# Koukyosyumei/MyZKP

Hardware: AMD Instinct MI355X
Metric: G1 MSM pairs/sec + NTT elems/sec at 2^20 and 2^24; bit-exact vs CPU (higher is better)
Workload: dtype u32x9 (29-bit limbs, 254-bit Montgomery); 1 GPU; KZG commit = BN254 G1 Pippenger MSM of 2^20 (scalar, point) pairs per GPU against a device-resident SRS (commit_kzg, kzg.rs:57-59); 17-bit signed windows (library default at this size), 15 window tables built once at upload; N GPUs = one MSM of N*2^20 pairs (BASELINE configs[2]/[3]); pairs_per_gpu=1048576, seed=332211571536, window_bits=17

## Files before the change

myzkp_amd/csrc/mzk_api.hip:

```cpp
#include <stdarg.h>
#include <stdlib.h>
#include <atomic>
#include "mzk_common.h"
#include "mzk_gl.h"

namespace mzk {

static thread_local char g_err[512] = "";
void set_error(const char* fmt, ...) {
  va_list ap;
  va_start(ap, fmt);
  vsnprintf(g_err, sizeof g_err, fmt, ap);
  va_end(ap);
}
void clear_error() { g_err[0] = 0; }
int hip_fail(hipError_t e, const char* what, const char* file, int line) {
  set_error("HIP error %d (%s) in %s at %s:%d", (int)e, hipGetErrorString(e), what, file, line);
  return MZK_E_HIP;
}

static std::atomic<uint64_t> g_owner{0};
static thread_local int t_depth = 0;
static thread_local char t_marker;
EntryGuard::EntryGuard() : ok(true), nested(false) {
// ... 1028 lines not shown
    const bool last = k == nc - 1;
    if (!last && g_table_budget && bytes > g_table_budget) continue;
    void* p = nullptr;
    if (n == 0 || dev_alloc(&p, bytes, "SRS handle") == MZK_OK) {
      h->d_points_mont = p; h->has_tables = cand[k].tables; h->window_bits = cand[k].bits; h->sets = cand[k].sets;
      return MZK_OK;
    }
  }
  set_error("SRS handle: the device has no %zu bytes left for the prepared points alone (idle workspace already released)", n * 128);
  return MZK_E_NOMEM;
}
int srs_fill(mzk_srs* h, const void* d_plain, hipStream_t s) {
  WsFrame ws("srs_fill");
  const size_t n = h->n;
  if (n == 0) return MZK_OK;
  if (!h->has_tables) return msm_prepare_points(d_plain, n, h->d_points_mont, (uint8_t*)h->d_points_mont + n * 64, s);
  void* d_mont;
  MZK_TRY(ws.get(WS_MSM_POINTS, n * 64, &d_mont));
  MZK_TRY(msm_prepare_points(d_plain, n, d_mont, nullptr, s));
  return msm_build_tables(d_mont, n, h->d_points_mont, h->window_bits * h->sets, s);
}
}

extern "C" {

int mzk_set_table_budget(size_t bytes) { g_table_budget = bytes; return MZK_OK; }
int mzk_set_workspace_budget(size_t bytes) {
  MZK_ENTER();
  g_ws_budget = bytes;
  if (bytes) {
// ... 486 lines not shown
```

myzkp_amd/csrc/mzk_common.h:

```cpp
#pragma once
#include <hip/hip_runtime.h>
#include <stdint.h>
#include <stddef.h>
#include <stdio.h>
#include <string.h>
#include <functional>
#include <string>
#include <vector>
#include "../../include/mzk.h"
#include "mzk_field.h"
#include "mzk_msm_plan.h"
#include "mzk_ws.h"

namespace mzk {

#ifdef MZK_TUNING
#include <stdlib.h>
static inline int tune_int(const char* name, int dflt) { const char* v = getenv(name); return v ? atoi(v) : dflt; } static inline const char* tune_str(const char* name) { return getenv(name); }
#else
static inline constexpr int tune_int(const char*, int dflt) { return dflt; }
static inline constexpr const char* tune_str(const char*) { return nullptr; }
#endif

void set_error(const char* fmt, ...);
// ... 167 lines not shown
  int k, K;
  size_t i0;
  size_t n_total;
  size_t n_alloc;
};
struct MsmChunk { const void* d_scalars; size_t i0, n; hipEvent_t ready; };
int msm_chunked_impl(const MsmChunk* chunks, int K, const void* d_points, size_t n_total, int point_kind, size_t table_stride, void* d_out,
                     bool out_partial_xyzz, hipStream_t s, const std::function<int(int)>* before_chunk = nullptr);
bool msm_chunkable(size_t n_total, int point_kind, size_t table_stride);
int msm_dev_impl(const void* d_scalars, const void* d_points, size_t n, int point_kind, size_t table_stride, void* d_out,
                 bool out_partial_xyzz, hipStream_t s, const std::function<int()>* points_ready = nullptr, const MsmChunkCtx* cc = nullptr);

bool msm_many_supported(int window_bits);
int msm_generic_window_bits(size_t n);
int msm_many_dev_impl(const void* d_scalars, size_t n, size_t stride_elems, size_t count, const void* d_tables, int c, size_t table_stride, void* d_out,
                      hipStream_t s);
constexpr size_t MSM_DIRECT_MAX_N = (size_t)1 << 14;
size_t msm_direct_bytes(size_t n, int c);
int msm_build_direct(const void* d_points_mont, size_t n, int c, void* d_direct, hipStream_t s);
int msm_direct_many_dev_impl(const void* d_scalars, size_t n, size_t stride_elems, size_t count, const void* d_direct, int c, size_t table_stride, void* d_out,
                             hipStream_t s);

int xyzz_batch_to_affine(const void* d_xyzz, size_t count, void* d_out, bool out_mont, hipStream_t s);
int msm_build_tables(const void* d_points_mont, size_t n, void* d_tables, int window_bits, hipStream_t s);
int msm_fold_partials_impl(const void* d_partials, int count, void* d_out_xy, hipStream_t s);
int msm_prepare_points(const void* d_points_plain, size_t n, void* d_points_mont, void* d_phi, hipStream_t s);
int msm_phi_points(const void* d_points_mont, size_t n, void* d_phi, hipStream_t s);
int synth_field_impl(int fid, uint64_t seed, size_t n, void* d_out, hipStream_t s);
int synth_g1_impl(uint64_t seed, size_t n, void* d_out, hipStream_t s);
int selftest_inv_wave_impl(uint64_t seed, size_t n, uint64_t* mismatches_host, hipStream_t s);
int selftest_row_ec_impl(uint64_t seed, size_t n, int dbl_reps, uint64_t* mismatches_host, hipStream_t s);
// ... 18 lines not shown
}

struct mzk_srs {
  void* d_points_mont;
  size_t n;
  bool has_tables;
  int window_bits;
  int ctx_index;
  int sets = 1;
  void* d_direct = nullptr;
  int direct_bits = 0;
  size_t direct_bytes = 0;
  mutable void* d_tables_wide = nullptr;
  mutable int wide_bits = 0;
  mutable size_t wide_bytes = 0;
  int kind() const { return has_tables ? (mzk::MSM_PTS_TABLES | (window_bits << 8) | (sets << 16)) : (int)mzk::MSM_PTS_MONT; }
  size_t table_rows() const { return has_tables ? (size_t)mzk::msm_table_rows(window_bits, sets) : 2; }
};

namespace mzk {
bool srs_many_capable(const mzk_srs* srs);
int msm_many_srs(const mzk_srs* srs, const void* d_scalars, size_t n, size_t stride_elems, size_t count, void* d_out, hipStream_t s,
                 size_t shift = 0);
bool kzg_open_many_supported(const mzk_srs* srs, size_t n);
int kzg_open_many_dev(const mzk_srs* srs, const void* d_coefs, size_t n, size_t count, const uint64_t* us_host, void* d_ys, void* d_ws_xy, hipStream_t s);
}
```

myzkp_amd/csrc/mzk_io.hip:

```cpp
#include <stdio.h>
#include <vector>
#include "mzk_common.h"

using namespace mzk;

namespace mzk {
int srs_alloc_layout(mzk_srs* h, int with_tables);
struct SrsFileHeader {
  char magic[8];
  uint32_t format;
  uint32_t flags;
  uint64_t n;
  uint32_t window_bits;
  uint32_t table_rows;
  uint64_t points_fnv1a;
  uint64_t tables_fnv1a;
  uint64_t reserved[2];
};
static_assert(sizeof(SrsFileHeader) == 64, "header layout");
static const char SRS_MAGIC[8] = {'M', 'Z', 'K', 'S', 'R', 'S', 0, 0};
static const size_t IO_CHUNK_POINTS = (size_t)1 << 19;

static uint64_t fnv1a(uint64_t h, const void* data, size_t len) {
  const uint8_t* p = (const uint8_t*)data;
// ... 83 lines not shown
  if (hash != h.points_fnv1a) { set_error("srs_load: checksum mismatch in %s (corrupted or truncated)", path); return MZK_E_IO; }
  const int want_bits = with_tables > 1 ? with_tables : msm_srs_window_bits(n);
  const bool use_stored = with_tables && h.format >= 2 && (h.flags & 1u) && (int)h.window_bits == want_bits &&
                          h.table_rows == (uint32_t)(msm_table_windows(want_bits) - 1) && n > 0;
  if (!use_stored) return mzk_srs_from_device_ex(d_plain, n, with_tables, out, s);
  WsGuard wsg(s);
  mzk_srs* hd = new mzk_srs{nullptr, n, false, 0, ctx().index};
  const size_t rows = (size_t)h.table_rows + 1;
  int rc = srs_alloc_layout(hd, with_tables);
  if (rc == MZK_OK && !(hd->has_tables && hd->sets == 1 && hd->window_bits == want_bits)) {
    mzk_srs_free(hd);
    return mzk_srs_from_device_ex(d_plain, n, with_tables, out, s);
  }
  if (rc != MZK_OK) { delete hd; return rc; }
  uint64_t thash = hash;
  if (rc == MZK_OK) rc = msm_prepare_points(d_plain, n, hd->d_points_mont, nullptr, s);
  for (size_t row = 1; rc == MZK_OK && row < rows; row++) {
    for (size_t at = 0; rc == MZK_OK && at < n; at += IO_CHUNK_POINTS) {
      const size_t m = n - at < IO_CHUNK_POINTS ? n - at : IO_CHUNK_POINTS;
      if (fread(host.data(), 64, m, fc.f) != m) { set_error("srs_load: %s is truncated (tables)", path); rc = MZK_E_IO; break; }
      thash = fnv1a_words(thash, host.data(), m * 64);
      if (hipMemcpyAsync((uint8_t*)hd->d_points_mont + (row * n + at) * 64, host.data(), m * 64, hipMemcpyHostToDevice, s) != hipSuccess ||
          hipStreamSynchronize(s) != hipSuccess) { set_error("srs_load: copy failed"); rc = MZK_E_HIP; }
    }
  }
  if (rc == MZK_OK && hipStreamSynchronize(s) != hipSuccess) rc = MZK_E_HIP;
  if (rc == MZK_OK && thash != h.tables_fnv1a) { set_error("srs_load: checksum mismatch in the window tables of %s (corrupted or stale)", path); rc = MZK_E_IO; }
  if (rc != MZK_OK) { mzk_srs_free(hd); return rc; }
  *out = hd;
  return MZK_OK;
// ... 24 lines not shown
```

myzkp_amd/csrc/mzk_msm.hip:

```cpp
#include <stdlib.h>
#include <type_traits>
#include "mzk_common.h"
#include "mzk_elem.h"
#include "mzk_ec.h"
#include "mzk_coop.h"
#include "mzk_row.h"
#include "mzk_glv.h"
#include "mzk_affine_wave.h"

namespace mzk {

static const MsmKnobs& msm_knobs() {
  static const MsmKnobs k = [] {
    const MsmKnobs d;
    return MsmKnobs{tune_int("MZK_GLV_C", d.glv_c), tune_int("MZK_SMALL_SCAN", d.small_scan), tune_int("MZK_SCAN_MAX_LOG", d.scan_max_log),
                    tune_int("MZK_ACC_SEG", d.acc_seg), tune_int("MZK_COARSE_LOG_20", d.coarse_log_20),
                    tune_int("MZK_COARSE_LOG_17", d.coarse_log_17), tune_int("MZK_PER_FINE", d.per_fine), tune_int("MZK_SORT_SCAN_FREE", d.sort_scan_free),
                    tune_int("MZK_COMBINE_WIDE_MIN_LOG", d.combine_wide_min_log)};
  }();
  return k;
}

int msm_generic_window_bits(size_t n) { return choose_shape_glv(n ? n : 1, msm_knobs().glv_c).c; }

// ... 704 lines not shown
    hipLaunchKernelGGL(k_scan_finish, dim3((unsigned)((n + 255) / 256 + 1)), dim3(256), 0, s, out, (const u32*)scratch, sb, n);
  } else {
    MZK_TRY(launch_exclusive_scan((const u32*)scratch, scratch, sb, scratch + sb + 2, s));
    hipLaunchKernelGGL(k_scan_add, dim3((unsigned)(n / 256 + 1)), dim3(256), 0, s, out, (const u32*)scratch, sb, n);
  }
  MZK_HIP(hipGetLastError());
  return MZK_OK;
}

constexpr u32 SEG_MIN = 8;
__device__ __forceinline__ u32 segment_length(u32 seg_host, u32 t_max, u32 total_entries) {
  if (t_max == 0) return seg_host;
  const u32 v = (total_entries + t_max - 1) / t_max;
  return v < SEG_MIN ? SEG_MIN : v;
}
template <bool SENT = false>
__global__ __launch_bounds__(256, 3) void k_seg_accumulate(const u32* __restrict__ points_mont, const u32* __restrict__ offsets,
                                                         const u32* __restrict__ entries, u32* __restrict__ slots, size_t nbuckets,
                                                         u32 seg_host, u32 t_max) {
  const size_t t = (size_t)blockIdx.x * blockDim.x + threadIdx.x;
  const u32 total_entries = offsets[nbuckets];
  u32 e0, e1;
  if (!seg_span(t, segment_length(seg_host, t_max, total_entries), total_entries, &e0, &e1)) return;
  const auto offset_at = [&](size_t b) __attribute__((always_inline)) { return offsets[b]; };
  Xyzz acc = xyzz_inf();
  u32 w[16];
  Affine pt;
  bool skip = false;
  seg_walk<SENT>(
      e0, e1, seg_first_bucket(offset_at, nbuckets, e0), nbuckets, [&](u32 e) __attribute__((always_inline)) { return entries[e]; }, offset_at,
      [&](u32 ref) __attribute__((always_inline)) {
        const size_t idx = ref & 0x7fffffffu;
        load_words8(points_mont + idx * 16, w);
        load_words8(points_mont + idx * 16 + 8, w + 8);
      },
      [&](u32 ent) __attribute__((always_inline)) {
#pragma unroll
        for (int k = 0; k < 16; k++) asm volatile("" : "+v"(w[k]));
        skip = affine_words_is_inf(w) || (SENT && ent == MANY_SENTINEL);
        pt = affine_load_mont(w);
      },
      [&](size_t b) __attribute__((always_inline)) {
        xyzz_gstore_raw(slots, t + b, acc);
        acc = xyzz_inf();
      },
      [&](u32, u32 ent, size_t) __attribute__((always_inline)) {
        if (!skip) acc = xyzz_madd_signed_with<FeAsm>(acc, pt, (ent >> 31) != 0);
      });
}
constexpr u32 HEAVY_SLOTS_SORT1 = 16;
__device__ __forceinline__ u32 bucket_end(const u32* __restrict__ offsets, const u32* __restrict__ tails, int lg_nb, size_t b) {
  if (tails && (b & (((size_t)1 << lg_nb) - 1)) == (((size_t)1 << lg_nb) - 1)) return tails[b >> lg_nb];
  return offsets[b + 1];
}
__device__ __forceinline__ bool defer_heavy(size_t b, size_t s0, size_t s1, u32 o1, u32* __restrict__ heavy, bool leader, u32 threshold = HEAVY_SLOTS) {
  if (s1 - s0 + 1 <= threshold) return false;
  if (leader) { const u32 i = atomicAdd(&heavy[0], 1u); heavy[HEAVY_HDR + 2 * i] = (u32)b; heavy[HEAVY_HDR + 2 * i + 1] = o1; }
  return true;
}
__global__ __launch_bounds__(128) void k_seg_combine_wide(const u32* __restrict__ slots, const u32* __restrict__ offsets,
                                                           u32* __restrict__ buckets, size_t nbuckets, u32 seg_host, u32* __restrict__ heavy, u32 t_max) {
  const size_t b = (size_t)blockIdx.x * blockDim.x + threadIdx.x;
  if (b >= nbuckets) return;
// ... 337 lines not shown
  }
  MZK_TRY(launch_reduce_tail_row(buckets, lgB, t_start, sets, wsum, 0, s));
  MZK_HIP(hipGetLastError());
  prof_end(s, MZK_PH_MSM_REDUCE);
  prof_begin(s, MZK_PH_MSM_COMBINE);
  MZK_TRY(launch_window_combine_row((const u32*)wsum, sets, horner_c, out_partial_xyzz ? 1 : 0, d_out, s));
  prof_end(s, MZK_PH_MSM_COMBINE);
  return MZK_OK;
}

int msm_prepare_points(const void* d_points_plain, size_t n, void* d_points_mont, void* d_phi, hipStream_t s) {
  if (n == 0) return MZK_OK;
  hipLaunchKernelGGL(k_prepare_points, dim3((unsigned)((n + 255) / 256)), dim3(256), 0, s, (const u32*)d_points_plain,
                     (u32*)d_points_mont, n, (u32*)d_phi);
  MZK_HIP(hipGetLastError());
  return MZK_OK;
}
int msm_points_to_plain(const void* d_points_mont, size_t n, void* d_points_plain, hipStream_t s) {
  if (n == 0) return MZK_OK;
  hipLaunchKernelGGL(k_points_to_plain, dim3((unsigned)((n + 255) / 256)), dim3(256), 0, s, (const u32*)d_points_mont, n, (u32*)d_points_plain);
  MZK_HIP(hipGetLastError());
  return MZK_OK;
}
int msm_phi_points(const void* d_points_mont, size_t n, void* d_phi, hipStream_t s) {
  if (n == 0) return MZK_OK;
  hipLaunchKernelGGL(k_phi_points, dim3((unsigned)((n + 255) / 256)), dim3(256), 0, s, (const u32*)d_points_mont, n, (u32*)d_phi);
  MZK_HIP(hipGetLastError());
  return MZK_OK;
}

// ... 175 lines not shown
      hipLaunchKernelGGL(k_wg_hist_prefix, dim3((unsigned)((P.NB + 255) / 256)), dim3(256), 0, s, wghist, P.nwg, (int)P.NB, counts);
      MZK_TRY(launch_exclusive_scan((const u32*)counts, offsets, P.NB, scan, s));
      hipLaunchKernelGGL(k_digits_scatter_lds, dim3(P.nwg), dim3(LDS_SORT_THREADS), lds, s, (const u32*)d_scalars, n, P.per_wg, P.L, (const u32*)offsets,
                         (const u32*)wghist, (const u32*)ranks, entries);
    } else {
      const unsigned nblk = (unsigned)((n + 255) / 256);
      MZK_HIP(hipMemsetAsync(counts, 0, P.NB * 4, s));
      hipLaunchKernelGGL(k_digits_count, dim3(nblk), dim3(256), 0, s, (const u32*)d_scalars, n, P.L, counts, ranks);
      MZK_TRY(launch_exclusive_scan((const u32*)counts, offsets, P.NB, scan, s));
      hipLaunchKernelGGL(k_digits_scatter, dim3(nblk), dim3(256), 0, s, (const u32*)d_scalars, n, P.L, offsets, ranks, entries);
    }
    MZK_HIP(hipGetLastError());
    prof_end(s, MZK_PH_MSM_SORT);
    MZK_TRY(prepare());
    prof_begin(s, MZK_PH_MSM_ACCUMULATE);
    hipLaunchKernelGGL(k_seg_accumulate<false>, dim3((unsigned)((P.T + 255) / 256)), dim3(256), 0, s, pts, offsets, entries, slots, P.NB, P.seg, P.t_max);
    prof_end(s, MZK_PH_MSM_ACCUMULATE);
    prof_begin(s, MZK_PH_MSM_SEG_COMBINE);
    if (P.combine_wide)
      hipLaunchKernelGGL(k_seg_combine_wide, dim3((unsigned)((P.NB + 127) / 128)), dim3(128), 0, s, slots, offsets, buckets, P.NB, P.seg, heavy, P.t_max);
    else
      hipLaunchKernelGGL(k_seg_combine, dim3((unsigned)((4 * P.NB + 127) / 128)), dim3(128), 0, s, slots, offsets, buckets, P.NB, P.seg, heavy, (const u32*)nullptr, 0, P.t_max);
    hipLaunchKernelGGL(k_seg_combine_heavy, dim3(HEAVY_GRID), dim3(HEAVY_THREADS), 0, s, (const u32*)slots, (const u32*)offsets, buckets, heavy, P.max_heavy);
    MZK_HIP(hipGetLastError());
    prof_end(s, MZK_PH_MSM_SEG_COMBINE);
    if (cc) return MZK_OK;
  }
  MZK_TRY(reduce_bucket_sets(buckets, P.lgB, P.red_windows, P.one_set, P.horner_c, wsum, (u32*)d_out, out_partial_xyzz, s));
  MZK_HIP(hipGetLastError());
  return MZK_OK;
}
// ... 140 lines not shown
  if (j + 1 == npoly && tid == 0) offsets[npoly * NB] = (u32)(npoly * cap);
  if (tid == 0) tails[j] = base + total;
  __syncthreads();
#pragma unroll
  for (int k = 0; k < SORT1_PER_LANE; k++) {
    const size_t i = tid + (size_t)k * SORT1_THREADS;
    if (i < n) walk_digits_merged<C>(w[k], table_stride, i, [&](int, u32 key, u32 payload) { stage[counter_inc_agg(hist, key)] = payload; });
  }
  __syncthreads();
  for (u32 e = tid; e < cap; e += SORT1_THREADS) entries[base + e] = (e < total) ? stage[e] : MANY_SENTINEL;
}

bool msm_many_supported(int window_bits) { return window_bits == 8 || (window_bits >= 10 && window_bits <= 13); }

int msm_many_dev_impl(const void* d_scalars, size_t n, size_t stride_elems, size_t count, const void* d_tables, int c, size_t table_stride, void* d_out,
                      hipStream_t s) {
  if (count == 0) return MZK_OK;
  if (!d_out || ((!d_scalars || !d_tables) && n)) { set_error("msm_many: null pointer"); return MZK_E_ARG; }
  if (!msm_many_supported(c)) { set_error("msm_many: window width %d has no grid-batched path", c); return MZK_E_ARG; }
  if (n == 0) {
    MZK_HIP(hipMemsetAsync(d_out, 0, count * 64, s));
    return MZK_OK;
  }
  const int nwin = msm_table_windows(c), lgB = c - 1;
  const size_t NB = (size_t)1 << lgB;
  if ((size_t)nwin * table_stride > ((size_t)1 << 31)) { set_error("msm_many: table rows exceed the 31-bit point references"); return MZK_E_ARG; }
  const int nch = (int)((n + MANY_CHUNK - 1) / MANY_CHUNK);
  size_t per_pass = ((size_t)1 << 21) / NB;
  const size_t by_coefs = (((size_t)1 << 22) + n - 1) / n;
  if (by_coefs < per_pass) per_pass = by_coefs;
  if (per_pass < 1) per_pass = 1;
// ... 43 lines not shown
        hipLaunchKernelGGL((k_many_sort1<C>), dim3(nwg), dim3(SORT1_THREADS), n * (size_t)nwin * 4, s, sc, n, stride_elems * 8, table_stride,       \
                           (u32)(n * (size_t)nwin), offs, cnt, entries, tails);                                                                           \
        break;                                                                                                                                       \
      }                                                                                                                                              \
      hipLaunchKernelGGL((k_many_count<C>), dim3(nwg), dim3(MANY_THREADS), 0, s, sc, n, stride_elems * 8, nch, offs);                                \
      MZK_TRY(launch_exclusive_scan((const u32*)offs, offs, ncnt, scan_tmp, s));                                                                     \
      hipLaunchKernelGGL((k_many_scatter<C>), dim3(nwg), dim3(MANY_THREADS), 0, s, sc, n, stride_elems * 8, nch, table_stride, (const u32*)offs,     \
                         nch > 1 ? compact : (u32*)nullptr, NBtot, entries);                                                                         \
      break;
    switch (c) { MZK_MANY_CASE(8) MZK_MANY_CASE(10) MZK_MANY_CASE(11) MZK_MANY_CASE(12) MZK_MANY_CASE(13) }
#undef MZK_MANY_CASE
    MZK_HIP(hipGetLastError());
    prof_end(s, MZK_PH_MSM_SORT);
    prof_begin(s, MZK_PH_MSM_ACCUMULATE);
    const u32 t_max = one_kernel_sort ? 0u : (u32)T;
    if (one_kernel_sort)
      hipLaunchKernelGGL(k_seg_accumulate<true>, dim3((unsigned)((T + 255) / 256)), dim3(256), 0, s, (const u32*)d_tables, (const u32*)compact, (const u32*)entries,
                         slots, NBtot, seg, t_max);
    else
      hipLaunchKernelGGL(k_seg_accumulate<false>, dim3((unsigned)((T + 255) / 256)), dim3(256), 0, s, (const u32*)d_tables, (const u32*)compact, (const u32*)entries,
                         slots, NBtot, seg, t_max);
    prof_end(s, MZK_PH_MSM_ACCUMULATE);
    prof_begin(s, MZK_PH_MSM_SEG_COMBINE);
    const unsigned cgrid = (unsigned)((4 * NBtot + 127) / 128);
    hipLaunchKernelGGL(k_seg_combine, dim3(cgrid), dim3(128), 0, s, slots, (const u32*)compact, buckets, NBtot, seg, heavy, (const u32*)tails, lgB, t_max);
    hipLaunchKernelGGL(k_seg_combine_heavy, dim3(HEAVY_GRID), dim3(HEAVY_THREADS), 0, s, (const u32*)slots, (const u32*)compact, buckets, heavy, max_heavy);
    MZK_HIP(hipGetLastError());
    prof_end(s, MZK_PH_MSM_SEG_COMBINE);
    prof_begin(s, MZK_PH_MSM_REDUCE);
    int t_start = 0;
    MZK_TRY(launch_halving_steps(buckets, lgB, (int)cnt, row_tail_max_ops(), &t_start, s));
    MZK_TRY(launch_reduce_tail_row(buckets, lgB, t_start, (int)cnt, out, 1, s));
    MZK_HIP(hipGetLastError());
    prof_end(s, MZK_PH_MSM_REDUCE);
  }
  return MZK_OK;
// ... 166 lines not shown
    if (!srs->d_tables_wide && srs->wide_bits == 0) {
      const size_t bytes = (size_t)msm_table_windows(MANY_WIDE_BITS) * srs->n * 64;
      const size_t own = (size_t)srs->n * 64 * srs->table_rows() + srs->direct_bytes;
      void* t = nullptr;
      const bool within_budget = table_budget_bytes() == 0 || own + bytes <= table_budget_bytes();
      if (within_budget && dev_alloc(&t, bytes, "wide window tables of the grid-batched pass") == MZK_OK) {
        const int rc = msm_build_tables(srs->d_points_mont, srs->n, t, MANY_WIDE_BITS, s);
        if (rc != MZK_OK) { (void)ws_hook_free(t); return rc; }
        srs->d_tables_wide = t; srs->wide_bits = MANY_WIDE_BITS; srs->wide_bytes = bytes;
      } else {
        srs->wide_bits = -1;
        if (within_budget) clear_error();
      }
    }
    if (srs->d_tables_wide)
      return msm_many_dev_impl(d_scalars, n, stride_elems, count, (const char*)srs->d_tables_wide + shift * 64, srs->wide_bits, srs->n, d_out, s);
  }
  return msm_many_dev_impl(d_scalars, n, stride_elems, count, (const char*)srs->d_points_mont + shift * 64, srs->window_bits, srs->n, d_out, s);
}

int msm_fold_partials_impl(const void* d_partials, int count, void* d_out_xy, hipStream_t s) {
  if (!d_partials || !d_out_xy || count < 0) { set_error("fold_partials: bad argument"); return MZK_E_ARG; }
  MZK_TRY(launch_fold_partials_row((const u32*)d_partials, count, (u32*)d_out_xy, s));
  return MZK_OK;
}

}

namespace mzk {
__device__ __forceinline__ u64 splitmix64(u64& s) {
  u64 z = (s += 0x9e3779b97f4a7c15ULL);
  z = (z ^ (z >> 30)) * 0xbf58476d1ce4e5b9ULL;
  z = (z ^ (z >> 27)) * 0x94d049bb133111ebULL;
// ... 91 lines not shown
```

myzkp_amd/csrc/mzk_msm_plan.h:

```cpp
#pragma once
#include <stddef.h>
#include <stdint.h>
#include <stdio.h>
#include "../../include/mzk.h"

namespace mzk {

enum { MSM_PTS_PLAIN = 0, MSM_PTS_MONT = 1, MSM_PTS_TABLES = 2 };
static inline int msm_table_windows(int c) { return 254 / c + 1; }
static inline int msm_table_rows(int c, int sets) { return 254 / (c * sets) + 1; }

constexpr int SCALAR_BITS = 254;
constexpr int MAX_WINDOWS = 32;
constexpr int GLV_MAG_BITS = 126;
constexpr int SLOT_WORDS = 36;
constexpr int ACC_RESIDENT_WAVES = 3;

struct DigitLayout {
  int c, nwin, merged;
  int sets;
  size_t table_stride;
  int glv;
  size_t phi_offset;
};
// ... 64 lines not shown
  int err = MZK_OK;
  char msg[192] = {};
  size_t n = 0;
  DigitLayout L{};
  int lgB = 0, red_windows = 0, horner_c = 0;
  size_t NB = 0, NBtot = 0;
  bool one_set = false, small_wide = false;
  MsmPath path = MsmPath::SmallSort;
  int cl = 0, F = 0, fb = 0, key_shift = 0, S = 0, nwg = 0;
  uint32_t fine_mask = 0, slice_cap = 0;
  unsigned fine_wgs = 0;
  size_t per_wg = 0;
  bool compact = false, coarse_free = false, fine_free = false, scatter_staged = false;
  int coarse_c = 0;
  uint32_t seg = 0, t_max = 0;
  size_t T = 0, nslots = 0, max_heavy = 0, slot_region_words = 0;
  bool combine_wide = false;
  MsmSizing own{}, alloc{};
  MsmWsBytes ws{}, ws_used{};
  MsmPlan& fail(const char* fmt, size_t a = 0, size_t b = 0, size_t c = 0) { err = MZK_E_ARG; snprintf(msg, sizeof msg, fmt, a, b, c); return *this; }
};

static inline size_t msm_slot_region_words(size_t T, size_t NB) {
  return ((T + NB + 1) * SLOT_WORDS + heavy_total_words((T + NB) / HEAVY_SLOTS + 1) + 3) & ~(size_t)3;
}
static inline MsmPlan& msm_sized(MsmPlan& P, size_t regions) {
  for (int u = 0; u < 2; u++) {
    const MsmSizing& z = u ? P.own : P.alloc;
    MsmWsBytes& w = u ? P.ws_used : P.ws;
    w.points = P.ws.points, w.out = P.ws.out;
    w.offsets = regions * (P.NBtot + 1) * 4;
    w.entries = regions * z.E * 4;
    w.buckets = regions * P.NB * 128;
    if (P.path == MsmPath::SmallScan || P.path == MsmPath::SmallSort) continue;
    const bool two = P.path == MsmPath::TwoLevel;
    w.counts = 2 * P.NBtot * 4;
    w.cursor = z.E * (two ? 8 : 4);
// ... 33 lines not shown
  if (!chunks && (scan_ok || n < (L.merged ? SMALL_MAX_N : SMALL_MAX_N - 1)) && P.NB <= SMALL_MAX_BUCKETS) {
    P.path = scan_ok ? MsmPath::SmallScan : MsmPath::SmallSort;
    P.small_wide = E_max / P.NB > 64;
    return msm_sized(P, 1);
  }
  const size_t ref_max = L.merged ? (size_t)msm_table_rows(L.c, L.sets) * table_stride : L.phi_offset + n;
  if (ref_max > ((size_t)1 << 31) || E_max >= ((size_t)1 << 32))
    return P.fail("msm: %zu pairs x %zu windows (table stride %zu) exceed the 31-bit point references / 32-bit entry offsets", n, (size_t)L.nwin, table_stride);

  const size_t resident_lanes = (size_t)num_cu * 4 * ACC_RESIDENT_WAVES * 64;
  size_t seg = (E_max + resident_lanes - 1) / resident_lanes;
  seg = kn.acc_seg > 0 ? (size_t)kn.acc_seg : seg < 16 ? 16 : seg;
  P.seg = (uint32_t)seg;
  P.T = P.own.T = (E_max + seg - 1) / seg;
  P.t_max = kn.acc_seg > 0 ? 0u : (uint32_t)P.T;
  P.nslots = P.T + P.NB + 1;
  P.max_heavy = (P.T + P.NB) / HEAVY_SLOTS + 1;
  P.combine_wide = P.NB >= ((size_t)1 << kn.combine_wide_min_log);
  const size_t T_seg = E_alloc / (kn.acc_seg > 0 ? (size_t)kn.acc_seg : 16) + 1;
  P.alloc.T = !chunks ? P.T : kn.acc_seg > 0 ? T_seg : (resident_lanes + 1 < T_seg ? resident_lanes + 1 : T_seg);
  P.slot_region_words = msm_slot_region_words(P.alloc.T, P.NB);

  const bool plain_merged = L.merged && L.sets == 1;
  P.cl = (plain_merged && L.c == 20 && kn.coarse_log_20 == 10) ? 10 : COARSE_LOG;
  if (plain_merged && L.c == 17 && kn.coarse_log_17 == 9 && COARSE_LOG == 8 && ref_max > ((size_t)1 << (31 - 8)) && ref_max <= ((size_t)1 << (31 - 7)))
    P.cl = 9;
  if (L.glv && P.NBtot > ((size_t)STAGE_F_MAX << COARSE_LOG)) P.cl = 10;
  const size_t cbins = (size_t)1 << P.cl;
  const bool two_level = (P.NBtot & (P.NBtot - 1)) == 0 && P.NBtot >= 4096 && (P.NBtot / cbins) <= (size_t)FINE_MAX &&
                         (n >= 4096 || (L.merged && P.NBtot > ((size_t)1 << 15)));
// ... 33 lines not shown
#if defined(__HIPCC__)
#define MZK_HD __host__ __device__ __forceinline__
#else
#define MZK_HD inline
#endif
constexpr uint32_t MANY_SENTINEL = 0xffffffffu;

MZK_HD bool seg_span(uint64_t t, uint32_t seg, uint32_t total, uint32_t* e0, uint32_t* e1) {
  const uint64_t e0w = t * seg;
  if (e0w >= total) return false;
  *e0 = (uint32_t)e0w;
  *e1 = (e0w + seg < total) ? (uint32_t)e0w + seg : total;
  return true;
}

template <int K, class Offset>
MZK_HD size_t seg_bucket_search(Offset offset_at, size_t nbuckets, uint32_t e) {
  size_t lo = 0, hi = nbuckets;
  while (hi - lo > 1) {
    const size_t step = (hi - lo + K - 1) / K;
    uint32_t v[K];
#if defined(__HIPCC__)
#pragma unroll
#endif
    for (int j = 1; j < K; j++) v[j] = offset_at(lo + j * step < hi ? lo + j * step : hi);
    size_t below = 0;
#if defined(__HIPCC__)
#pragma unroll
#endif
    for (int j = 1; j < K; j++) below += v[j] <= e ? 1 : 0;
    lo += below * step;
    if (lo + step < hi) hi = lo + step;
  }
  return lo;
}
template <class Offset>
MZK_HD size_t seg_first_bucket(Offset offset_at, size_t nbuckets, uint32_t e) {
  return nbuckets <= ((size_t)1 << 20) ? seg_bucket_search<16>(offset_at, nbuckets, e) : seg_bucket_search<32>(offset_at, nbuckets, e);
}

template <bool SENT, class Entry, class Offset, class IssueRow, class TakeRow, class Flush, class Add>
MZK_HD void seg_walk(uint32_t e0, uint32_t e1, size_t b, size_t nbuckets, Entry entry_at, Offset offset_at, IssueRow issue_row, TakeRow take_row,
                     Flush flush, Add add) {
  const auto row_ref = [](uint32_t ent) { return (SENT && ent == MANY_SENTINEL) ? 0u : ent; };
  const auto end_after_next = [&](size_t bb) { return offset_at(bb + 2 <= nbuckets ? bb + 2 : nbuckets); };
  uint32_t ent = entry_at(e0);
  uint32_t ent1 = entry_at(e1 - e0 > 1 ? e0 + 1 : e0);
  issue_row(row_ref(ent));
  uint32_t bend = offset_at(b + 1), bend1 = end_after_next(b);
  for (uint32_t e = e0; e < e1; e++) {
    take_row(ent);
    const uint32_t ent2 = entry_at(e1 - e > 2 ? e + 2 : e1 - 1);
    issue_row(row_ref(ent1));
    if (e >= bend) {
      flush(b);
      b++, bend = bend1;
      while (e >= bend) b++, bend = offset_at(b + 1);
      bend1 = end_after_next(b);
    }
    add(e, ent, b);
    ent = ent1, ent1 = ent2;
  }
  flush(b);
}

typedef uint32_t u32;
typedef uint64_t u64;
MZK_HD u32 raw_window(const u32* w, int win, int c) {
  const int bit = win * c;
  if (bit >= 256) return 0;
  const int k = bit >> 5, s = bit & 31;
  u64 v = w[k];
  if (k + 1 < 8) v |= (u64)w[k + 1] << 32;
  return (u32)(v >> s) & ((1u << c) - 1u);
}
template <class Emit>
MZK_HD void walk_digits_whole(const u32* w, const DigitLayout& L, size_t i, Emit emit) {
  const int c = L.c;
// ... 59 lines not shown
```

Before: 775.0 million pairs/s.

## Specialize segment accumulate for finite SRS points, fresh buckets, and 32-bit indexing

Adds a one-time device check at SRS upload that records whether any point is at infinity. When none are, the accumulate kernel is instantiated without the per-point infinity test. The accumulator now starts from the first affine point instead of doing a mixed add onto infinity, and empty buckets are stored as zeros directly. A narrow 32-bit indexing variant is used when sizes allow, to cut address arithmetic. The cost is eight kernel instantiations, an extra host sync during SRS fill, and some register-pinning asm.

Result: no change. 776.6 million pairs/s (median of 6 runs) (+0.2%).

```diff
diff --git a/myzkp_amd/csrc/mzk_api.hip b/myzkp_amd/csrc/mzk_api.hip
--- a/myzkp_amd/csrc/mzk_api.hip
+++ b/myzkp_amd/csrc/mzk_api.hip
@@ -1066,6 +1066,7 @@
   WsFrame ws("srs_fill");
   const size_t n = h->n;
   if (n == 0) return MZK_OK;
+  MZK_TRY(msm_points_finite(d_plain, n, &h->finite, s));
   if (!h->has_tables) return msm_prepare_points(d_plain, n, h->d_points_mont, (uint8_t*)h->d_points_mont + n * 64, s);
   void* d_mont;
   MZK_TRY(ws.get(WS_MSM_POINTS, n * 64, &d_mont));
diff --git a/myzkp_amd/csrc/mzk_common.h b/myzkp_amd/csrc/mzk_common.h
--- a/myzkp_amd/csrc/mzk_common.h
+++ b/myzkp_amd/csrc/mzk_common.h
@@ -205,7 +205,8 @@
 bool msm_many_supported(int window_bits);
 int msm_generic_window_bits(size_t n);
 int msm_many_dev_impl(const void* d_scalars, size_t n, size_t stride_elems, size_t count, const void* d_tables, int c, size_t table_stride, void* d_out,
-                      hipStream_t s);
+                      hipStream_t s, bool rows_finite = false);
+int msm_points_finite(const void* d_points_plain, size_t n, bool* finite, hipStream_t s);
 constexpr size_t MSM_DIRECT_MAX_N = (size_t)1 << 14;
 size_t msm_direct_bytes(size_t n, int c);
 int msm_build_direct(const void* d_points_mont, size_t n, int c, void* d_direct, hipStream_t s);
@@ -254,7 +255,10 @@
   mutable void* d_tables_wide = nullptr;
   mutable int wide_bits = 0;
   mutable size_t wide_bytes = 0;
-  int kind() const { return has_tables ? (mzk::MSM_PTS_TABLES | (window_bits << 8) | (sets << 16)) : (int)mzk::MSM_PTS_MONT; }
+  bool finite = false;
+  int kind() const {
+    return (has_tables ? (mzk::MSM_PTS_TABLES | (window_bits << 8) | (sets << 16)) : (int)mzk::MSM_PTS_MONT) | (finite ? (int)mzk::MSM_PTS_FINITE : 0);
+  }
   size_t table_rows() const { return has_tables ? (size_t)mzk::msm_table_rows(window_bits, sets) : 2; }
 };
 
diff --git a/myzkp_amd/csrc/mzk_ec_acc.h b/myzkp_amd/csrc/mzk_ec_acc.h
--- /dev/null
+++ b/myzkp_amd/csrc/mzk_ec_acc.h
@@ -0,0 +1,13 @@
+#pragma once
+#include "mzk_ec.h"
+
+namespace mzk {
+
+MZK_HD Xyzz xyzz_acc_first(const Affine& q, bool neg) { return xyzz_from_affine(neg ? affine_neg(q) : q); }
+
+template <template <class> class A> MZK_HD void xyzz_acc_step(Xyzz& acc, bool fresh, const Affine& q, bool neg) {
+  if (fresh) acc = xyzz_acc_first(q, neg);
+  else acc = xyzz_madd_signed_with<A>(acc, q, neg);
+}
+
+}
diff --git a/myzkp_amd/csrc/mzk_io.hip b/myzkp_amd/csrc/mzk_io.hip
--- a/myzkp_amd/csrc/mzk_io.hip
+++ b/myzkp_amd/csrc/mzk_io.hip
@@ -121,6 +121,7 @@
   }
   if (rc != MZK_OK) { delete hd; return rc; }
   uint64_t thash = hash;
+  if (rc == MZK_OK) rc = msm_points_finite(d_plain, n, &hd->finite, s);
   if (rc == MZK_OK) rc = msm_prepare_points(d_plain, n, hd->d_points_mont, nullptr, s);
   for (size_t row = 1; rc == MZK_OK && row < rows; row++) {
     for (size_t at = 0; rc == MZK_OK && at < n; at += IO_CHUNK_POINTS) {
diff --git a/myzkp_amd/csrc/mzk_msm.hip b/myzkp_amd/csrc/mzk_msm.hip
--- a/myzkp_amd/csrc/mzk_msm.hip
+++ b/myzkp_amd/csrc/mzk_msm.hip
@@ -3,6 +3,7 @@
 #include "mzk_common.h"
 #include "mzk_elem.h"
 #include "mzk_ec.h"
+#include "mzk_ec_acc.h"
 #include "mzk_coop.h"
 #include "mzk_row.h"
 #include "mzk_glv.h"
@@ -742,39 +743,77 @@
   const u32 v = (total_entries + t_max - 1) / t_max;
   return v < SEG_MIN ? SEG_MIN : v;
 }
-template <bool SENT = false>
+template <bool NARROW, class T> __device__ __forceinline__ const T* acc_at(const T* __restrict__ base, u32 index) {
+  if (NARROW) return reinterpret_cast<const T*>(reinterpret_cast<const char*>(base) + (u32)(index * (u32)sizeof(T)));
+  return base + index;
+}
+__device__ __forceinline__ void xyzz_gstore_raw_live(u32* __restrict__ g, size_t idx, const Xyzz& p) {
+  uint4* p4 = reinterpret_cast<uint4*>(g + idx * SLOT_WORDS);
+  u32 w[SLOT_WORDS];
+#pragma unroll
+  for (int i = 0; i < FqParams::L; i++) { w[i] = p.X.l[i]; w[9 + i] = p.Y.l[i]; w[18 + i] = p.ZZ.l[i]; w[27 + i] = p.ZZZ.l[i]; }
+#pragma unroll
+  for (int q = 0; q < SLOT_WORDS / 4; q++) p4[q] = make_uint4(w[4 * q], w[4 * q + 1], w[4 * q + 2], w[4 * q + 3]);
+}
+__device__ __forceinline__ void xyzz_gstore_raw_inf(u32* __restrict__ g, size_t idx) {
+  uint4* p4 = reinterpret_cast<uint4*>(g + idx * SLOT_WORDS);
+#pragma unroll
+  for (int q = 0; q < SLOT_WORDS / 4; q++) p4[q] = make_uint4(0u, 0u, 0u, 0u);
+}
+template <bool SENT = false, bool MAYINF = true, bool NARROW = false>
 __global__ __launch_bounds__(256, 3) void k_seg_accumulate(const u32* __restrict__ points_mont, const u32* __restrict__ offsets,
                                                          const u32* __restrict__ entries, u32* __restrict__ slots, size_t nbuckets,
                                                          u32 seg_host, u32 t_max) {
+  typedef typename std::conditional<NARROW, u32, size_t>::type Idx;
   const size_t t = (size_t)blockIdx.x * blockDim.x + threadIdx.x;
   const u32 total_entries = offsets[nbuckets];
   u32 e0, e1;
   if (!seg_span(t, segment_length(seg_host, t_max, total_entries), total_entries, &e0, &e1)) return;
-  const auto offset_at = [&](size_t b) __attribute__((always_inline)) { return offsets[b]; };
-  Xyzz acc = xyzz_inf();
+  const auto offset_at = [&](Idx b) __attribute__((always_inline)) { return NARROW ? *acc_at<NARROW>(offsets, (u32)b) : offsets[b]; };
+  Xyzz acc;
   u32 w[16];
   Affine pt;
+  pt.x = fe_zero<FqParams>(), pt.y = fe_zero<FqParams>();
   bool skip = false;
-  seg_walk<SENT>(
-      e0, e1, seg_first_bucket(offset_at, nbuckets, e0), nbuckets, [&](u32 e) __attribute__((always_inline)) { return entries[e]; }, offset_at,
+  seg_walk_acc<SENT>(
+      e0, e1, seg_first_bucket(offset_at, (Idx)nbuckets, e0), (Idx)nbuckets, [&](u32 e) __attribute__((always_inline)) { return *acc_at<NARROW>(entries, e); },
+      offset_at,
       [&](u32 ref) __attribute__((always_inline)) {
-        const size_t idx = ref & 0x7fffffffu;
-        load_words8(points_mont + idx * 16, w);
-        load_words8(points_mont + idx * 16 + 8, w + 8);
+        asm volatile("" : "+v"(ref) : "v"(pt.x.l[0]), "v"(pt.x.l[1]), "v"(pt.x.l[2]), "v"(pt.x.l[3]), "v"(pt.x.l[4]), "v"(pt.x.l[5]), "v"(pt.x.l[6]), "v"(pt.x.l[7]),
+                     "v"(pt.x.l[8]), "v"(pt.y.l[0]), "v"(pt.y.l[1]), "v"(pt.y.l[2]), "v"(pt.y.l[3]), "v"(pt.y.l[4]), "v"(pt.y.l[5]), "v"(pt.y.l[6]), "v"(pt.y.l[7]),
+                     "v"(pt.y.l[8]));
+        const u32* row = NARROW ? acc_at<NARROW>(points_mont, (ref & 0x7fffffffu) * 16u) : points_mont + (size_t)(ref & 0x7fffffffu) * 16;
+        load_words8(row, w);
+        load_words8(row + 8, w + 8);
       },
       [&](u32 ent) __attribute__((always_inline)) {
 #pragma unroll
         for (int k = 0; k < 16; k++) asm volatile("" : "+v"(w[k]));
-        skip = affine_words_is_inf(w) || (SENT && ent == MANY_SENTINEL);
+        skip = (MAYINF && affine_words_is_inf(w)) || (SENT && ent == MANY_SENTINEL);
         pt = affine_load_mont(w);
       },
-      [&](size_t b) __attribute__((always_inline)) {
-        xyzz_gstore_raw(slots, t + b, acc);
-        acc = xyzz_inf();
+      [&](Idx b, bool fresh) __attribute__((always_inline)) {
+        if (fresh) {
+          xyzz_gstore_raw_inf(slots, t + b);
+          asm volatile("" ::: "memory");
+        } else {
+          xyzz_gstore_raw_live(slots, t + b, acc);
+        }
       },
-      [&](u32, u32 ent, size_t) __attribute__((always_inline)) {
-        if (!skip) acc = xyzz_madd_signed_with<FeAsm>(acc, pt, (ent >> 31) != 0);
+      [&](u32, u32 ent, Idx, bool fresh) __attribute__((always_inline)) {
+        if ((MAYINF || SENT) && skip) return fresh;
+        xyzz_acc_step<FeAsm>(acc, fresh, pt, (ent >> 31) != 0);
+        return false;
       });
+}
+static void launch_seg_accumulate(bool sent, bool mayinf, bool narrow, size_t T, hipStream_t s, const u32* points_mont, const u32* offsets, const u32* entries,
+                                  u32* slots, size_t nbuckets, u32 seg, u32 t_max) {
+  const dim3 grid((unsigned)((T + 255) / 256)), block(256);
+#define MZK_ACC_CASE(S, M, N) \
+  if (sent == S && mayinf == M && narrow == N) hipLaunchKernelGGL((k_seg_accumulate<S, M, N>), grid, block, 0, s, points_mont, offsets, entries, slots, nbuckets, seg, t_max)
+  MZK_ACC_CASE(false, false, false); MZK_ACC_CASE(false, false, true); MZK_ACC_CASE(false, true, false); MZK_ACC_CASE(false, true, true);
+  MZK_ACC_CASE(true, false, false); MZK_ACC_CASE(true, false, true); MZK_ACC_CASE(true, true, false); MZK_ACC_CASE(true, true, true);
+#undef MZK_ACC_CASE
 }
 constexpr u32 HEAVY_SLOTS_SORT1 = 16;
 __device__ __forceinline__ u32 bucket_end(const u32* __restrict__ offsets, const u32* __restrict__ tails, int lg_nb, size_t b) {
@@ -1142,6 +1181,33 @@
   hipLaunchKernelGGL(k_prepare_points, dim3((unsigned)((n + 255) / 256)), dim3(256), 0, s, (const u32*)d_points_plain,
                      (u32*)d_points_mont, n, (u32*)d_phi);
   MZK_HIP(hipGetLastError());
+  return MZK_OK;
+}
+__global__ void k_points_any_infinity(const u32* __restrict__ in, size_t n, u32* __restrict__ flag) {
+  const size_t i = (size_t)blockIdx.x * blockDim.x + threadIdx.x;
+  bool bad = false;
+  if (i < n) {
+    u32 y[8];
+    load_words8(in + i * 16 + 8, y);
+    u32 acc = 0;
+#pragma unroll
+    for (int k = 0; k < 8; k++) acc |= y[k];
+    bad = acc == 0;
+  }
+  if (__syncthreads_or(bad) && threadIdx.x == 0) atomicOr(flag, 1u);
+}
+int msm_points_finite(const void* d_points_plain, size_t n, bool* finite, hipStream_t s) {
+  *finite = false;
+  if (n == 0) return MZK_OK;
+  DevMem flag;
+  MZK_TRY(flag.alloc(4, "SRS handle: infinity flag"));
+  MZK_HIP(hipMemsetAsync(flag.get(), 0, 4, s));
+  hipLaunchKernelGGL(k_points_any_infinity, dim3((unsigned)((n + 255) / 256)), dim3(256), 0, s, (const u32*)d_points_plain, n, flag.as<u32>());
+  MZK_HIP(hipGetLastError());
+  u32 any = 1;
+  MZK_HIP(hipMemcpyAsync(&any, flag.get(), 4, hipMemcpyDeviceToHost, s));
+  MZK_HIP(hipStreamSynchronize(s));
+  *finite = any == 0;
   return MZK_OK;
 }
 int msm_points_to_plain(const void* d_points_mont, size_t n, void* d_points_plain, hipStream_t s) {
@@ -1347,7 +1413,7 @@
     prof_end(s, MZK_PH_MSM_SORT);
     MZK_TRY(prepare());
     prof_begin(s, MZK_PH_MSM_ACCUMULATE);
-    hipLaunchKernelGGL(k_seg_accumulate<false>, dim3((unsigned)((P.T + 255) / 256)), dim3(256), 0, s, pts, offsets, entries, slots, P.NB, P.seg, P.t_max);
+    launch_seg_accumulate(false, !P.rows_finite, P.acc_narrow, P.T, s, pts, offsets, entries, slots, P.NB, P.seg, P.t_max);
     prof_end(s, MZK_PH_MSM_ACCUMULATE);
     prof_begin(s, MZK_PH_MSM_SEG_COMBINE);
     if (P.combine_wide)
@@ -1518,7 +1584,7 @@
 bool msm_many_supported(int window_bits) { return window_bits == 8 || (window_bits >= 10 && window_bits <= 13); }
 
 int msm_many_dev_impl(const void* d_scalars, size_t n, size_t stride_elems, size_t count, const void* d_tables, int c, size_t table_stride, void* d_out,
-                      hipStream_t s) {
+                      hipStream_t s, bool rows_finite) {
   if (count == 0) return MZK_OK;
   if (!d_out || ((!d_scalars || !d_tables) && n)) { set_error("msm_many: null pointer"); return MZK_E_ARG; }
   if (!msm_many_supported(c)) { set_error("msm_many: window width %d has no grid-batched path", c); return MZK_E_ARG; }
@@ -1592,12 +1658,8 @@
     prof_end(s, MZK_PH_MSM_SORT);
     prof_begin(s, MZK_PH_MSM_ACCUMULATE);
     const u32 t_max = one_kernel_sort ? 0u : (u32)T;
-    if (one_kernel_sort)
-      hipLaunchKernelGGL(k_seg_accumulate<true>, dim3((unsigned)((T + 255) / 256)), dim3(256), 0, s, (const u32*)d_tables, (const u32*)compact, (const u32*)entries,
-                         slots, NBtot, seg, t_max);
-    else
-      hipLaunchKernelGGL(k_seg_accumulate<false>, dim3((unsigned)((T + 255) / 256)), dim3(256), 0, s, (const u32*)d_tables, (const u32*)compact, (const u32*)entries,
-                         slots, NBtot, seg, t_max);
+    launch_seg_accumulate(one_kernel_sort, !rows_finite, seg_narrow_ok((size_t)nwin * table_stride, E_max, NBtot), T, s, (const u32*)d_tables, (const u32*)compact,
+                          (const u32*)entries, slots, NBtot, seg, t_max);
     prof_end(s, MZK_PH_MSM_ACCUMULATE);
     prof_begin(s, MZK_PH_MSM_SEG_COMBINE);
     const unsigned cgrid = (unsigned)((4 * NBtot + 127) / 128);
@@ -1794,9 +1856,9 @@
       }
     }
     if (srs->d_tables_wide)
-      return msm_many_dev_impl(d_scalars, n, stride_elems, count, (const char*)srs->d_tables_wide + shift * 64, srs->wide_bits, srs->n, d_out, s);
-  }
-  return msm_many_dev_impl(d_scalars, n, stride_elems, count, (const char*)srs->d_points_mont + shift * 64, srs->window_bits, srs->n, d_out, s);
+      return msm_many_dev_impl(d_scalars, n, stride_elems, count, (const char*)srs->d_tables_wide + shift * 64, srs->wide_bits, srs->n, d_out, s, srs->finite);
+  }
+  return msm_many_dev_impl(d_scalars, n, stride_elems, count, (const char*)srs->d_points_mont + shift * 64, srs->window_bits, srs->n, d_out, s, srs->finite);
 }
 
 int msm_fold_partials_impl(const void* d_partials, int count, void* d_out_xy, hipStream_t s) {
diff --git a/myzkp_amd/csrc/mzk_msm_plan.h b/myzkp_amd/csrc/mzk_msm_plan.h
--- a/myzkp_amd/csrc/mzk_msm_plan.h
+++ b/myzkp_amd/csrc/mzk_msm_plan.h
@@ -7,6 +7,7 @@
 namespace mzk {
 
 enum { MSM_PTS_PLAIN = 0, MSM_PTS_MONT = 1, MSM_PTS_TABLES = 2 };
+enum { MSM_PTS_FINITE = 1 << 24 };
 static inline int msm_table_windows(int c) { return 254 / c + 1; }
 static inline int msm_table_rows(int c, int sets) { return 254 / (c * sets) + 1; }
 
@@ -102,6 +103,8 @@
   bool compact = false, coarse_free = false, fine_free = false, scatter_staged = false;
   int coarse_c = 0;
   uint32_t seg = 0, t_max = 0;
+  bool rows_finite = false;
+  bool acc_narrow = false;
   size_t T = 0, nslots = 0, max_heavy = 0, slot_region_words = 0;
   bool combine_wide = false;
   MsmSizing own{}, alloc{};
@@ -109,6 +112,9 @@
   MsmPlan& fail(const char* fmt, size_t a = 0, size_t b = 0, size_t c = 0) { err = MZK_E_ARG; snprintf(msg, sizeof msg, fmt, a, b, c); return *this; }
 };
 
+static inline bool seg_narrow_ok(size_t rows, size_t entries, size_t nbuckets) {
+  return rows <= ((size_t)1 << 26) && entries < ((size_t)1 << 30) && nbuckets < ((size_t)1 << 30);
+}
 static inline size_t msm_slot_region_words(size_t T, size_t NB) {
   return ((T + NB + 1) * SLOT_WORDS + heavy_total_words((T + NB) / HEAVY_SLOTS + 1) + 3) & ~(size_t)3;
 }
@@ -172,6 +178,8 @@
   P.seg = (uint32_t)seg;
   P.T = P.own.T = (E_max + seg - 1) / seg;
   P.t_max = kn.acc_seg > 0 ? 0u : (uint32_t)P.T;
+  P.rows_finite = kind != MSM_PTS_PLAIN && (point_kind & MSM_PTS_FINITE) != 0;
+  P.acc_narrow = seg_narrow_ok(ref_max, E_max, P.NB);
   P.nslots = P.T + P.NB + 1;
   P.max_heavy = (P.T + P.NB) / HEAVY_SLOTS + 1;
   P.combine_wide = P.NB >= ((size_t)1 << kn.combine_wide_min_log);
@@ -235,17 +243,17 @@
   return true;
 }
 
-template <int K, class Offset>
-MZK_HD size_t seg_bucket_search(Offset offset_at, size_t nbuckets, uint32_t e) {
-  size_t lo = 0, hi = nbuckets;
+template <int K, class Idx, class Offset>
+MZK_HD Idx seg_bucket_search(Offset offset_at, Idx nbuckets, uint32_t e) {
+  Idx lo = 0, hi = nbuckets;
   while (hi - lo > 1) {
-    const size_t step = (hi - lo + K - 1) / K;
+    const Idx step = (hi - lo + K - 1) / K;
     uint32_t v[K];
 #if defined(__HIPCC__)
 #pragma unroll
 #endif
-    for (int j = 1; j < K; j++) v[j] = offset_at(lo + j * step < hi ? lo + j * step : hi);
-    size_t below = 0;
+    for (int j = 1; j < K; j++) v[j] = offset_at(lo + (Idx)j * step < hi ? lo + (Idx)j * step : hi);
+    Idx below = 0;
 #if defined(__HIPCC__)
 #pragma unroll
 #endif
@@ -255,34 +263,45 @@
   }
   return lo;
 }
-template <class Offset>
-MZK_HD size_t seg_first_bucket(Offset offset_at, size_t nbuckets, uint32_t e) {
-  return nbuckets <= ((size_t)1 << 20) ? seg_bucket_search<16>(offset_at, nbuckets, e) : seg_bucket_search<32>(offset_at, nbuckets, e);
-}
-
-template <bool SENT, class Entry, class Offset, class IssueRow, class TakeRow, class Flush, class Add>
-MZK_HD void seg_walk(uint32_t e0, uint32_t e1, size_t b, size_t nbuckets, Entry entry_at, Offset offset_at, IssueRow issue_row, TakeRow take_row,
-                     Flush flush, Add add) {
+template <class Idx, class Offset>
+MZK_HD Idx seg_first_bucket(Offset offset_at, Idx nbuckets, uint32_t e) {
+  return nbuckets <= ((Idx)1 << 20) ? seg_bucket_search<16>(offset_at, nbuckets, e) : seg_bucket_search<32>(offset_at, nbuckets, e);
+}
+
+template <bool SENT, class Idx, class Entry, class Offset, class IssueRow, class TakeRow, class Flush, class Add>
+MZK_HD void seg_walk_acc(uint32_t e0, uint32_t e1, Idx b, Idx nbuckets, Entry entry_at, Offset offset_at, IssueRow issue_row, TakeRow take_row,
+                         Flush flush, Add add) {
   const auto row_ref = [](uint32_t ent) { return (SENT && ent == MANY_SENTINEL) ? 0u : ent; };
-  const auto end_after_next = [&](size_t bb) { return offset_at(bb + 2 <= nbuckets ? bb + 2 : nbuckets); };
+  const auto end_after_next = [&](Idx bb) { return offset_at(bb + 2 <= nbuckets ? bb + 2 : nbuckets); };
   uint32_t ent = entry_at(e0);
   uint32_t ent1 = entry_at(e1 - e0 > 1 ? e0 + 1 : e0);
   issue_row(row_ref(ent));
   uint32_t bend = offset_at(b + 1), bend1 = end_after_next(b);
+  bool fresh = true;
+  const uint32_t last = e1 - 1;
   for (uint32_t e = e0; e < e1; e++) {
     take_row(ent);
-    const uint32_t ent2 = entry_at(e1 - e > 2 ? e + 2 : e1 - 1);
+    const uint32_t ahead = last - e;
+    const uint32_t ent2 = entry_at(e + (ahead < 2 ? ahead : 2u));
     issue_row(row_ref(ent1));
     if (e >= bend) {
-      flush(b);
+      flush(b, fresh);
+      fresh = true;
       b++, bend = bend1;
       while (e >= bend) b++, bend = offset_at(b + 1);
       bend1 = end_after_next(b);
     }
-    add(e, ent, b);
+    fresh = add(e, ent, b, fresh);
     ent = ent1, ent1 = ent2;
   }
-  flush(b);
+  flush(b, fresh);
+}
+template <bool SENT, class Entry, class Offset, class IssueRow, class TakeRow, class Flush, class Add>
+MZK_HD void seg_walk(uint32_t e0, uint32_t e1, size_t b, size_t nbuckets, Entry entry_at, Offset offset_at, IssueRow issue_row, TakeRow take_row,
+                     Flush flush, Add add) {
+  seg_walk_acc<SENT, size_t>(
+      e0, e1, b, nbuckets, entry_at, offset_at, issue_row, take_row, [&](size_t bb, bool) { flush(bb); },
+      [&](uint32_t e, uint32_t ent, size_t bb, bool) { add(e, ent, bb); return false; });
 }
 
 typedef uint32_t u32;
```
